# andr345/frtm-vos

Measured on AMD Instinct MI355X. Metric: segmented frames/sec/GPU (480p, ResNet101, full CG iters), higher is better.
Workload: dtype f32

## Files before the change

frtm-vos_amd/_hip.py:

```python
import ctypes
import os

import torch

_HERE = os.path.dirname(os.path.abspath(__file__))
LIB_PATH = os.path.join(_HERE, 'libfrtm_hip.so')

P, I, F, D = ctypes.c_void_p, ctypes.c_int, ctypes.c_float, ctypes.c_double


class ConvDesc(ctypes.Structure):
    _fields_ = [(k, I) for k in ('B', 'Cin', 'Hin', 'Win', 'Cout', 'ksize', 'stride', 'pad',
                                 'relu', 'out_transposed', 'splitk', 'tile', 'w_layout', 'ws_elems', 'w_pitch')]


SIGNATURES = {
    'frtm_last_error': (ctypes.c_char_p, []),
    'frtm_version': (I, []),
    'frtm_device_info': (I, [P]),
    'frtm_pixel_weights': (I, [P, I, I, I, I, F, P, P, P]),
    'frtm_normal_build': (I, [P, I, P, I, I, I, I, I, F, P, I, P, P, P, P, P]),
    'frtm_memory_next_slot': (I, [P, I, F, I, P, P, I, P]),
    'frtm_memory_insert': (I, [P, P, I, P, P]),
    'frtm_filter_scores': (I, [P, P, I, I, I, I, P, I, P]),
    'frtm_stencil': (I, [P, P, P, P, I, I, I, P, P]),
    'frtm_filter_wgrad': (I, [P, P, I, I, I, I, I, P, P]),
    'frtm_filter_wgrad_parts': (I, [I, I]),
    'frtm_filter_wgrad_parts_hw': (I, [I, I, I]),
# ... 52 lines not shown
    'frtm_backbone_set_lanes': (I, [P, I]),
    'frtm_backbone_generation': (I, [P]),
    'frtm_backbone_set_winograd': (I, [P, I]),
    'frtm_backbone_set_winograd4': (I, [P, I]),
    'frtm_backbone_set_precision': (I, [P, I]),
    'frtm_merge_masks': (I, [P, I, I, P]),
    'frtm_merge_masks_frames': (I, [P, I, I, I, P]),
    'frtm_count_above': (I, [P, I, I, F, P, P]),
    'frtm_track_merge': (I, [P, I, I, I, P, P, P, I, P, F, P]),
    'frtm_filter_scores_pitched': (I, [P, P, I, I, I, I, P, I, I, P]),
    'frtm_bilinear_resize': (I, [P, I, I, I, P, I, I, P]),
    'frtm_tse_inject': (I, [P, P, P, P, I, I, I, I, I, I, I, P, P]),
    'frtm_cab_combine': (I, [P, P, P, I, I, I, I, I, I, I, P, P]),
    'frtm_pyrup2x': (I, [P, I, I, I, P, P]),
    'frtm_plane_mean': (I, [P, I, I, P, P]),
    'frtm_conv_wgrad_ws_elems': (ctypes.c_size_t, [I, I, I, I, I, I]),
    'frtm_conv_wgrad': (I, [P, P, I, I, I, I, I, I, P, P, P, ctypes.c_size_t, P]),
    'frtm_bn_stats': (I, [P, I, I, I, F, F, I, P, P, P, P, P, P]),
    'frtm_bn_apply_relu': (I, [P, P, P, P, P, I, I, I, P, P]),
    'frtm_bn_relu_backward': (I, [P, P, P, P, P, P, I, I, I, I, P, P, P, P, P]),
    'frtm_relu_backward': (I, [P, P, ctypes.c_size_t, P, P]),
    'frtm_pyrup2x_backward': (I, [P, I, I, I, P, P, P]),
    'frtm_bilinear_backward': (I, [P, I, I, I, I, I, P, P, P]),
    'frtm_cab_backward_reduce': (I, [P, P, I, I, P, P, P]),
    'frtm_cab_gate_backward': (I, [P, P, P, P, P, P, P, P, I, I, P, P, P, P, P, P, P]),
    'frtm_cab_backward_shallow': (I, [P, P, P, I, I, P, P]),
    'frtm_add_plane': (I, [P, P, F, I, I, P]),
    'frtm_shift9': (I, [P, I, I, I, P, P]),
    'frtm_cab_gate': (I, [P, P, I, P, P, P, P, I, I, P, P]),
    'frtm_project_tail': (I, [P, I, I, I, I, P, P, I, I, P, P]),
# ... 256 lines not shown
```

frtm-vos_amd/build.py:

```python
import os
import subprocess
import sys

HERE = os.path.dirname(os.path.abspath(__file__))
CSRC = os.path.join(HERE, 'csrc')
LIB = os.path.join(HERE, 'libfrtm_hip.so')
SOURCES = ['target_model.hip', 'cg_persistent.hip', 'joint_persistent.hip', 'joint_fit.hip', 'wide_maps.hip', 'conv_igemm.hip', 'conv_gemm32.hip', 'conv_wino.hip', 'conv_wino4.hip', 'conv_bf16x3.hip', 'backbone.hip', 'image_ops.hip', 'refiner_ops.hip', 'refiner_train.hip', 'telea_host.hip', 'jf_eval.hip', 'train_step.hip', 'frame_resize.hip']
HIPCC = os.environ.get('HIPCC', '/opt/rocm/bin/hipcc')
FLAGS = ['--offload-arch=gfx950', '-O3', '-std=c++17', '-fPIC', '-Wall', '-Wno-unused-function']
if os.environ.get('FRTM_BUILD_ABLATE'):
    FLAGS.append('-DFRTM_DEBUG_ABLATE')


def _stale(target, deps):
    if not os.path.exists(target):
        return True
    t = os.path.getmtime(target)
    return any(os.path.getmtime(d) > t for d in deps)


def build(force=False, verbose=True):
    headers = [os.path.join(CSRC, 'frtm_common.h'), os.path.join(CSRC, 'conv_common.h'), os.path.join(CSRC, 'resident_grid.h'), os.path.join(os.path.dirname(HERE), 'include', 'frtm_hip.h'), __file__]
    objs = []
    for src in SOURCES:
# ... 21 lines not shown
```

frtm-vos_amd/csrc/backbone.hip:

```cpp
#include <vector>
#include <algorithm>
#include <mutex>
#include <chrono>
#include <cstdio>
#include "frtm_common.h"
#include "../../include/frtm_hip.h"

void frtm_conv_plan(int M, int Ntot, int nchunks, int vec1x1, int* tile, int* splitk);

struct ConvL {
  int Cout, Cin, ks, stride, pad;
  float* wT = nullptr; float* scale = nullptr; float* shift = nullptr; int* ktab = nullptr;
  float* wW = nullptr;
  float* wW4 = nullptr;
  float* wW6 = nullptr;
  float* wB = nullptr;
  bool loaded = false;
  int layout = 0;
  int plan_tile = 0, plan_splitk = 0;
};
struct BlockL { int conv[3]; int nconv; int ds; };

struct Lane {
  float* buf[6] = {nullptr, nullptr, nullptr, nullptr, nullptr, nullptr};
// ... 132 lines not shown
static bool bf16x3_packs(const ConvL& c) { return bf16x3_eligible(c) && c.Cin == 512 && c.Cout == 2048; }
static bool bf16x3_route(const ConvL& c, int B, int Ho, int Wo) { return bf16x3_packs(c) && (long)B * Ho * Wo >= 3240; }

static int pack_bf16x3(ConvL& c, hipStream_t st) {
  if (!c.wB) FRTM_HIP(hipMalloc((void**)&c.wB, FRTM_CONV_BF16X3_ELEMS(c.Cout, c.Cin) * sizeof(float)));
  return frtm_bf16x3_pack(c.wT, c.Cout, c.Cin, 1, (c.Cout + 31) / 32 * 32, c.wB, st);
}

static int run_conv(frtm_backbone* bb, Lane& ln, int idx, int B, int Hin, int Win, const float* in, const float* residual, int relu,
                    float* out, int* Ho, int* Wo, hipStream_t st, int pad_override = -1) {
  ConvL& c = bb->convs[idx];
  if (!c.loaded) { frtm_set_error("backbone: conv %d has no weights (call frtm_backbone_set_conv)", idx); return FRTM_ERR_STATE; }
  const int pad = pad_override >= 0 ? pad_override : c.pad;
  frtm_conv_desc d;
  d.B = B; d.Cin = c.Cin; d.Hin = Hin; d.Win = Win; d.Cout = c.Cout; d.ksize = c.ks; d.stride = c.stride; d.pad = pad;
  d.relu = relu; d.out_transposed = 0; d.splitk = 0; d.tile = 0; d.w_pitch = 0; d.w_layout = c.layout; d.ws_elems = 0;
  *Ho = (Hin + 2 * pad - c.ks) / c.stride + 1;
  *Wo = (Win + 2 * pad - c.ks) / c.stride + 1;
  {
    const size_t out_elems = (size_t)c.Cout * B * (*Ho) * (*Wo);
    const size_t w = std::min((size_t)FRTM_CONV_MAX_SPLITK * out_elems, (size_t)16 * 1024 * 1024);
    int rc = ensure(bb, &ln.ws, &ln.ws_elems, std::max(w, out_elems * 2));
    if (rc) return rc;
  }
  d.ws_elems = (int)std::min<size_t>(ln.ws_elems, 0x7fffffff);
  bb->last_launches += 1;
  bb->last_flops += 2.0 * c.Cout * (double)B * (*Ho) * (*Wo) * c.Cin * c.ks * c.ks;
  if (c.wW4 && bb->use_winograd && bb->use_winograd4) {
    int best_m = 0; long best_cost = 0, best_T = 0, best_Tp = 0;
    for (int m : {6, 4}) {
      if (m == 6 && (bb->use_winograd4 < 2 || !c.wW6)) continue;
// ... 418 lines not shown
```

frtm-vos_amd/csrc/conv_common.h:

```cpp
#pragma once
#include "frtm_common.h"

typedef float f32x4 __attribute__((ext_vector_type(4)));
typedef float f32x4u __attribute__((ext_vector_type(4), aligned(4)));

struct FastDiv { unsigned m = 1, s = 0; };
static inline FastDiv fast_div(unsigned d) {
  FastDiv f;
  unsigned s = 0;
  while ((1ull << s) < d) ++s;
  f.s = s;
  f.m = (unsigned)(((((1ull << s) - d) << 32) / d) + 1);
  return f;
}

struct ConvParams {
  const float* in; const float* wT; const int* ktab; const float* scale; const float* shift;
  const float* residual; float* out; float* ws;
  int B, Cin, Hin, Win, M, Mp, Ho, Wo, K, stride, pad;
  int Npix, Ntot, relu, out_transposed, splitk, chunks_per_split, nchunks;
  unsigned in_bytes, w_bytes;
  int w_img_stride = 0;
  int epi_pre = 1;
  FastDiv dNpix, dWo, dMt;
  FastDiv dA, dB;
  int ntiles = 0;
};

#ifdef __HIPCC__
__device__ __forceinline__ int fdiv(int n, FastDiv f) { return (int)((__umulhi((unsigned)n, f.m) + (unsigned)n) >> f.s); }
#endif
static inline void fill_divs(ConvParams& p, int bm) {
  p.dNpix = fast_div((unsigned)p.Npix);
  p.dWo = fast_div((unsigned)p.Wo);
  p.dMt = fast_div((unsigned)((p.M + bm - 1) / bm));
}

void conv_trace_reset();
void conv_trace(const char* fmt, ...) __attribute__((format(printf, 1, 2)));

constexpr int BK = 32;
// ... 41 lines not shown
```

frtm-vos_amd/csrc/conv_igemm.hip:

```cpp
#include <algorithm>
#include <atomic>
#include <cstdarg>
#include <cstdio>
#include <cstdlib>
#include "frtm_common.h"
#include "../../include/frtm_hip.h"

#include "conv_common.h"

int frtm_wino_pack(const float* w_oihw, int Cout, int Cin, float* wT, hipStream_t st);
int frtm_wino_launch(ConvParams& p, int variant, hipStream_t st);
int frtm_wino4_pack(const float* w_oihw, int Cout, int Cin, float* U, int m, hipStream_t st);
int frtm_wino4_launch(const ConvParams& p, float* ws, size_t ws_elems, int tile, int m, hipStream_t st);
int frtm_g32_launch(const ConvParams& p, int tile, hipStream_t st);
int frtm_bf16x3_pack(const float* src, int Cout, int Cin, int sm, int sk, float* out, hipStream_t st);
int frtm_bf16x3_launch(ConvParams p, hipStream_t st);

static thread_local char t_conv_trace[256];
static thread_local int t_conv_trace_len = 0;
void conv_trace_reset() { t_conv_trace_len = 0; t_conv_trace[0] = 0; }
void conv_trace(const char* fmt, ...) {
  char name[96];
  va_list ap;
  va_start(ap, fmt);
// ... 884 lines not shown
                const float* residual, float* out, float* workspace, frtm_stream_t stream) {
  conv_trace_reset();
  FRTM_CHECK_ARG(d && in && wT && out, "frtm_conv2d: null pointer");
  FRTM_CHECK_ARG(d->B > 0 && d->Cin > 0 && d->Cout > 0 && d->ksize > 0 && d->stride > 0 && d->pad >= 0, "frtm_conv2d: bad shape");
  FRTM_CHECK_ARG((scale == nullptr) == (shift == nullptr), "frtm_conv2d: scale and shift go together");
  ConvParams p;
  p.in = in; p.wT = wT; p.ktab = ktab; p.scale = scale; p.shift = shift; p.residual = residual; p.out = out; p.ws = workspace;
  p.B = d->B; p.Cin = d->Cin; p.Hin = d->Hin; p.Win = d->Win; p.M = d->Cout; p.stride = d->stride; p.pad = d->pad;
  p.Ho = (d->Hin + 2 * d->pad - d->ksize) / d->stride + 1;
  p.Wo = (d->Win + 2 * d->pad - d->ksize) / d->stride + 1;
  FRTM_CHECK_ARG(p.Ho > 0 && p.Wo > 0, "frtm_conv2d: empty output");
  p.K = d->Cin * d->ksize * d->ksize;
  p.Npix = p.Ho * p.Wo;
  p.Ntot = d->B * p.Npix;
  p.relu = d->relu; p.out_transposed = d->out_transposed;
  static const bool no_epipre = getenv("FRTM_NO_EPIPRE") != nullptr;
  p.epi_pre = no_epipre ? 0 : 1;
  p.nchunks = ceil_div(p.K, BK);
  p.Mp = (p.M + 31) / 32 * 32;
  size_t w_bytes = (size_t)p.nchunks * BK * p.Mp * 4;
  if (d->w_pitch > 0) {
    FRTM_CHECK_ARG(d->w_pitch >= p.M && d->w_pitch % 4 == 0 && ((size_t)wT) % 16 == 0,
                   "frtm_conv2d: w_pitch must be >= Cout, a multiple of 4, and wT 16-byte aligned (got %d)", d->w_pitch);
    p.Mp = d->w_pitch;
    w_bytes = (size_t)p.K * p.Mp * 4;
  }
  const size_t in_bytes = (size_t)d->B * d->Cin * d->Hin * d->Win * 4;
  FRTM_CHECK_ARG(in_bytes < 0x7fffffffull && w_bytes < 0x7fffffffull, "frtm_conv2d: tensor too large for 32-bit buffer offsets");
  p.in_bytes = (unsigned)in_bytes; p.w_bytes = (unsigned)w_bytes;
  if (d->w_layout == FRTM_WLAYOUT_WINO3X3) {
// ... 122 lines not shown
```

frtm-vos_amd/csrc/conv_wino.hip:

```cpp
#include <algorithm>
#include <cstdlib>
#include <type_traits>
#include "frtm_common.h"
#include "../../include/frtm_hip.h"
#include "conv_common.h"

#ifdef FRTM_DEBUG_TRACE
__device__ unsigned long long* g_ktw_buf = nullptr;
__device__ unsigned g_ktw_cap = 0;
__device__ unsigned g_ktw_n[288];
#define KTW_STAMP(i) do { if (threadIdx.x == 0) kt[i] = wall_clock64(); } while (0)
#else
#define KTW_STAMP(i) do { } while (0)
#endif
#if defined(FRTM_DEBUG_TRACE) && FRTM_DEBUG_TRACE >= 2
#define KTW_IN(i) do { __builtin_amdgcn_sched_barrier(0); const unsigned long long t_ = __builtin_amdgcn_s_memrealtime(); kt_in[i] += t_ - kt_last; kt_last = t_; __builtin_amdgcn_sched_barrier(0); } while (0)
#define KTW_EPI(i) do { __builtin_amdgcn_sched_barrier(0); ke[i] = __builtin_amdgcn_s_memrealtime(); __builtin_amdgcn_sched_barrier(0); } while (0)
#else
#define KTW_IN(i) do { } while (0)
#define KTW_EPI(i) do { } while (0)
#endif

constexpr int WCI = 8;
constexpr int WBM = 32;
// ... 172 lines not shown
  for (; kc + 4 <= nch; kc += 2) {
    chunk(kc, st, I0{}, I2{}); st = st == 2 ? 0 : st + 1;
    chunk(kc + 1, st, I1{}, I2{}); st = st == 2 ? 0 : st + 1;
  }
  chunk(kc, st, I0{}, I1{}); st = st == 2 ? 0 : st + 1;
  chunk(kc + 1, st, I1{}, I0{});

  constexpr int TW = BW / 2, TH = BH / 2, TILES = TW * TH;
  const int tx = tid % TW, ty = (tid / TW) % TH, cq = tid / TILES;
  const int ej = FN == 2 ? (TALL ? ty >> 2 : tx >> 2) : 0, eli = (ty & 3) * 4 + (tx & 3);
  const int mm0 = m0 + cq * CQ;
  const int xx = x0 + 2 * tx, yy0 = y0 + 2 * ty;
  const bool two = xx + 1 < p.Wo;
  const size_t img_off = (size_t)img * p.M * p.Npix;
  const unsigned out_bytes = (unsigned)p.M * (unsigned)p.Npix * 4u;
  const __amdgpu_buffer_rsrc_t rout = __builtin_amdgcn_make_buffer_rsrc((void*)(p.out + img_off), 0, (int)out_bytes, 0x00020000);
  const __amdgpu_buffer_rsrc_t rres = __builtin_amdgcn_make_buffer_rsrc(p.residual ? (void*)(p.residual + img_off) : (void*)p.out, 0,
                                                                        p.residual ? (int)out_bytes : 0, 0x00020000);
  const bool pairs = (p.Wo & 1) == 0 && (((size_t)p.out) % 8 == 0) && (!p.residual || ((size_t)p.residual) % 8 == 0);
  unsigned eo[CQ][2];
#pragma unroll
  for (int c = 0; c < CQ; ++c)
#pragma unroll
    for (int a = 0; a < 2; ++a)
      eo[c][a] = (mm0 + c < p.M && yy0 + a < p.Ho && xx < p.Wo) ? (unsigned)(((mm0 + c) * p.Npix + (yy0 + a) * p.Wo + xx) * 4) : OOB;
  f32x2 rv[CQ][2];
  __builtin_amdgcn_sched_barrier(0);
  if (pairs) {
#pragma unroll
    for (int c = 0; c < CQ; ++c)
#pragma unroll
      for (int a = 0; a < 2; ++a) rv[c][a] = __builtin_bit_cast(f32x2, __builtin_amdgcn_raw_buffer_load_b64(rres, (int)eo[c][a], 0, 0));
  } else {
#pragma unroll
// ... 100 lines not shown
  }
}

int frtm_wino_pack(const float* w_oihw, int Cout, int Cin, float* wT, hipStream_t st) {
  const size_t total = (size_t)ceil_div(Cin, WCI) * WCI * ceil_div(Cout, WBM) * WBM;
  k_pack_weights_wino<<<(int)std::min((total + 255) / 256, (size_t)2048), 256, 0, st>>>(w_oihw, Cout, Cin, wT);
  conv_trace("k_pack_weights_wino");
  FRTM_LAUNCH_CHECK();
  return FRTM_OK;
}

int frtm_wino_launch(ConvParams& p, int variant, hipStream_t st) {
  p.nchunks = ceil_div(p.Cin, WCI);
  p.w_bytes = (unsigned)((size_t)p.nchunks * ceil_div(p.M, WBM) * WFRAG * 4);
  p.splitk = 1;
  const int mt = ceil_div(p.M, WBM);
  auto padded = [&](int bh, int bw) { return (long)ceil_div(p.Ho, bh) * bh * ceil_div(p.Wo, bw) * bw; };
  if (variant == 0) {
    const long a1 = padded(8, 8), a2 = padded(8, 16), a3 = padded(16, 8);
    variant = a2 <= a3 ? 2 : 3;
    const long a = variant == 2 ? a2 : a3;
    const long blocks2 = (long)p.B * (a / 128) * mt;
    if (mt > 2 || a * 100 > a1 * 115 || blocks2 < (mt == 1 ? 512 : 1024)) variant = 1;
  }
  p.dMt = fast_div((unsigned)mt);
  { const int bh = variant == 3 ? 16 : 8, bw = variant == 2 ? 16 : 8;
    p.dA = fast_div((unsigned)(ceil_div(p.Ho, bh) * ceil_div(p.Wo, bw))); p.dB = fast_div((unsigned)ceil_div(p.Wo, bw)); }
  if (variant == 2) {
    k_conv3x3_wino<2, 0, 3><<<p.B * ceil_div(p.Ho, 8) * ceil_div(p.Wo, 16) * mt, 256, 0, st>>>(p);
    conv_trace("k_conv3x3_wino<2,0,3>");
// ... 27 lines not shown
```

frtm-vos_amd/model/seg_network.py:

```python
import torch
from torch import nn
from torch.nn import functional as F

from .. import _hip as H
from .. import ops
from ..lib.utils import conv, relu, interpolate


def _bicubic_phase(d):
    x = (d + torch.arange(-1, 3, dtype=torch.float32)).abs()
    a = -0.75
    near = (a + 2) * x ** 3 - (a + 3) * x ** 2 + 1
    far = a * x ** 3 - 5 * a * x ** 2 + 8 * a * x - 4 * a
    return torch.where(x < 1, near, torch.where(x < 2, far, torch.zeros_like(x)))


_SIDE = {}


def _shared_side_stream(dev):
    key = torch.device(dev).index
    if key not in _SIDE:
        _SIDE[key] = torch.cuda.Stream(device=dev)
    return _SIDE[key]
# ... 112 lines not shown
        self.RRB2 = nn.ModuleDict()
        for L, fc in self.ft_channels.items():
            self.TSE[L] = TSE(fc, in_channels, out_channels)
            self.RRB1[L] = RRB(out_channels, use_bn=use_bn)
            self.CAB[L] = CAB(out_channels, L == 'layer5')
            self.RRB2[L] = RRB(out_channels, use_bn=use_bn)
        self.project = _HEADS[upsampler](out_channels)
        self.use_graphs = False
        self.parallel_eager = True
        self._graphs = {}
        self._pack_key = None
        self.use_winograd = True
        self.fuse_tail = True
        self.mix_taps = True
        self.parallel_levels = True
        self._side = None
        self._pool = None
        self._uses = {}
        self.capture_after = 1

    def invalidate(self):
        self._pack_key = None
        self._graphs = {}

    def __setattr__(self, name, value):
        if isinstance(value, nn.Module) and '_pack_key' in self.__dict__:
            self.invalidate()
        super().__setattr__(name, value)

    def _apply(self, fn, *a, **k):
        self.invalidate()
# ... 79 lines not shown

    def _packed(self):
        if getattr(self, '_pack_key', None) is not None:
            return self._pack
        key = tuple((p.data_ptr(), p._version) for p in list(self.parameters()) + list(self.buffers()))
        dev = next(self.parameters()).device

        def cv(m, scale=None, shift=None, relu_=False):
            wT, ktab, lay = ops.pack_weights(m.weight.data)
            cout = m.weight.shape[0]
            if shift is None:
                shift = m.bias.data.float() if m.bias is not None else None
            if shift is not None and scale is None:
                scale = torch.ones(cout, device=dev)
            wW = ops.pack_weights(m.weight.data, wino=True)[0] if m.weight.shape[2] == 3 else None
            return dict(wT=wT, ktab=ktab, lay=lay, cout=cout, k=m.weight.shape[2], scale=None if scale is None else scale.contiguous(),
                        shift=None if shift is None else shift.contiguous(), relu=relu_, wW=wW)

        def rrb(m):
            first = m.bblock[0]
            if isinstance(m.bblock[1], nn.BatchNorm2d):
                bn = m.bblock[1]
                sc = (bn.weight / torch.sqrt(bn.running_var + bn.eps)).data.float()
                sh = (sc * (first.bias.data - bn.running_mean) + bn.bias.data).float()
            else:
                sc, sh = None, None
            return dict(c1=cv(m.conv1x1), b0=cv(first, sc, sh, True), b1=cv(m.bblock[-1], relu_=True))

        P = {}
        for L in self.ft_channels:
            t = self.TSE[L]
            w0 = t.transform[0].weight.data
# ... 10 lines not shown
        if isinstance(pj, Upsampler):
            kind = 'bicubic'
        elif isinstance(pj, BackwardCompatibleUpsampler):
            kind = 'compat'
        else:
            raise TypeError('SegNetwork: no HIP path for the head %s' % type(pj).__name__)
        P['project'] = dict(kind=kind, c1=cv(pj.conv1, relu_=True), w2=pj.conv2.weight.data.contiguous(), b2=pj.conv2.bias.data,
                            eye9=torch.eye(9, device=dev).contiguous())
        self._pack, self._pack_key = P, key
        return P

    def _conv(self, x, c, residual=None):
        if c.get('wW') is not None and self.use_winograd:
            n, _, hh, ww = x.shape
            if n * ((hh + 7) // 8) * ((ww + 7) // 8) * ((c['cout'] + 31) // 32) >= 512:
                return ops.conv2d(x, c['wW'], c['cout'], 3, 1, 1, scale=c['scale'], shift=c['shift'], residual=residual,
                                  relu=c['relu'], splitk=1, w_layout=2)
        return ops.conv2d(x, c['wT'], c['cout'], c['k'], 1, c['k'] // 2, ktab=c['ktab'], scale=c['scale'], shift=c['shift'],
                          residual=residual, relu=c['relu'], w_layout=c['lay'])

    def _rrb_hip(self, x, r):
        a = self._conv(x, r['c1'])
        return self._conv(self._conv(a, r['b0']), r['b1'], residual=a)

    @staticmethod
    def _mean(x):
        n, c, hh, ww = x.shape
        out = torch.empty(n, c, device=x.device)
        H.call('frtm_plane_mean', H.ptr(x), n * c, hh * ww, H.ptr(out))
        return out

    def _branch(self, L, p, ft, scores, deepest):
        N, _, sh, sw = scores.shape
        F_, Hh, Ww = ft.shape[0], ft.shape[-2], ft.shape[-1]
# ... 9 lines not shown
        return r, self._mean(r), pool0, (h, base, t0, t)

    def _forward_hip(self, scores, features, image_size, side_streams=None):
        P = self._packed()
        scores = scores.float().contiguous()
        n = scores.shape[0]
        frames = features[next(iter(self.ft_channels))].shape[0]
        if n % frames != 0:
            raise ValueError('scores (%d samples) must hold the same number of objects for each of the %d frames' % (n, frames))
        group = n // frames
        dev = scores.device
        levels = list(self.ft_channels)
        cur = torch.cuda.current_stream()
        keep, br = [], {}
        self._capture_events = []

        def order(waiter, waited):
            ev = torch.cuda.Event()
            ev.record(waited)
            waiter.wait_event(ev)
            self._capture_events.append(ev)
        for st in set(side_streams or []):
            order(st, cur)
        for i, L in enumerate(levels):
            ft = features[L].contiguous()
            st = side_streams[i] if (side_streams and i < len(side_streams)) else None
            if st is None:
                br[L] = self._branch(L, P[L], ft, scores, i == 0)
            else:
                with torch.cuda.stream(st):
                    br[L] = self._branch(L, P[L], ft, scores, i == 0)
        x, pool0 = None, br[levels[0]][2]
        for i, L in enumerate(levels):
            p = P[L]
            st = side_streams[i] if (side_streams and i < len(side_streams)) else None
            if st is not None:
                order(cur, st)
            r, sp, _, tmp = br[L]
            keep.append(tmp)
            Hh, Ww = r.shape[-2:]
            dp = pool0 if x is None else self._mean(x)
            gate = torch.empty(n, r.shape[1], device=dev)
            H.call('frtm_cab_gate', H.ptr(sp), H.ptr(dp), group if x is None else 0, H.ptr(p['cab_w1']), H.ptr(p['cab_b1']),
                   H.ptr(p['cab_w2']), H.ptr(p['cab_b2']), n, r.shape[1], H.ptr(gate))
            out = torch.empty_like(r)
            if x is None:
                H.call('frtm_cab_combine', H.ptr(r), H.ptr(gate), H.ptr(pool0), n, r.shape[1], 1, 1, group, Hh, Ww, H.ptr(out))
            else:
                H.call('frtm_cab_combine', H.ptr(r), H.ptr(gate), H.ptr(x), n, r.shape[1], x.shape[2], x.shape[3], 0, Hh, Ww, H.ptr(out))
            keep.append((x, gate, out, dp))
            x = self._rrb_hip(out, p['rrb2'])
        pj = P['project']
        if pj['kind'] == 'bicubic':
            return self._head_bicubic(x, pj, image_size)
        c, hh, ww = x.shape[1:]
        u1 = torch.empty(n, c, 2 * hh, 2 * ww, device=dev)
        H.call('frtm_pyrup2x', H.ptr(x), n * c, hh, ww, H.ptr(u1))
        y = self._conv(u1, pj['c1'])
        c2 = y.shape[1]
        Ho, Wo = int(image_size[-2]), int(image_size[-1])
        if self.fuse_tail and int(18 * 4.0 * hh / Ho) + 3 <= 22 and int(66 * 4.0 * ww / Wo) + 3 <= 76:
            out = torch.empty(n, 1, Ho, Wo, device=dev)
            if self.mix_taps and c2 > 9:
                ym = torch.empty(n, 9, 2 * hh, 2 * ww, device=dev)
                H.call('frtm_tap_mix', H.ptr(y), n, c2, 4 * hh * ww, H.ptr(pj['w2']), H.ptr(ym))
                H.call('frtm_project_tail', H.ptr(ym), n, 9, 2 * hh, 2 * ww, H.ptr(pj['eye9']), H.ptr(pj['b2']), Ho, Wo, H.ptr(out))
# ... 39 lines not shown
```

frtm-vos_amd/ops.py:

```python
import ctypes

import torch

from . import _hip as H

_workspaces = {}


def workspace(device, elems):
    if torch.cuda.is_current_stream_capturing():
        return torch.empty(int(elems), device=device, dtype=torch.float32)
    key = (device, H.stream())
    w = _workspaces.get(key)
    if w is None or w.numel() < elems:
        w = torch.empty(int(elems), device=device, dtype=torch.float32)
        _workspaces[key] = w
    return w


def padded_rows(K):
    return (K + 31) // 32 * 32


def padded_cols(M):
# ... 13 lines not shown
        return wT, None, 5
    layout = 4 if wino6 else 3 if wino4 else 2 if wino else (1 if (halo if halo is not None else k == 3) else 0)
    rows = 64 * padded_rows(Cin) if layout == 4 else 36 * padded_rows(Cin) if layout == 3 else max(padded_rows(Cin * k * k), (Cin + 7) // 8 * 72) if layout != 2 else (Cin + 7) // 8 * 128
    wT = torch.zeros(rows, padded_cols(Cout), device=w.device)
    ktab = torch.empty(Cin * k * k * 3, device=w.device, dtype=torch.int32) if (k > 1 and layout == 0) else None
    H.call('frtm_conv_pack_weights', H.ptr(w), Cout, Cin, k, layout, H.ptr(wT), H.ptr(ktab))
    return wT, ktab, layout


def wino4_workspace(B, Cin, Cout, Hh, Ww, device, m=4):
    tiles = (B * ((Hh + m - 1) // m) * ((Ww + m - 1) // m) + 63) // 64 * 64
    return torch.empty((m + 2) ** 2 * (Cin + Cout) * tiles, device=device)


def conv2d(x, wT, Cout, ksize=1, stride=1, pad=0, ktab=None, scale=None, shift=None, residual=None, relu=False,
           out=None, out_transposed=False, splitk=0, tile=0, shape=None, w_pitch=0, w_layout=0, ws=None):
    B, Cin, Hin, Win = shape if shape is not None else x.shape
    Ho = (Hin + 2 * pad - ksize) // stride + 1
    Wo = (Win + 2 * pad - ksize) // stride + 1
    if out is None:
        out = torch.empty((B, Ho * Wo, Cout) if out_transposed else (B, Cout, Ho, Wo), device=x.device, dtype=torch.float32)
    out_elems = Cout * B * Ho * Wo
    if ws is None and splitk != 1:
        ws = workspace(x.device, min(32 * out_elems, max(2 * out_elems, 1 << 24)))
    d = H.ConvDesc(B, Cin, Hin, Win, Cout, ksize, stride, pad, int(relu), int(out_transposed), int(splitk), int(tile), int(w_layout),
                   0 if ws is None else min(ws.numel(), 0x7fffffff), int(w_pitch))
    H.call('frtm_conv2d', ctypes.byref(d), H.ptr(x), H.ptr(wT), H.ptr(ktab), H.ptr(scale), H.ptr(shift),
           H.ptr(residual), H.ptr(out), H.ptr(ws))
    return out


def filter_scores(X, f, out=None, accumulate=False, n=None, interleave=None):
    N = X.shape[0] if n is None else n
    C, h, w = X.shape[1:]
    if interleave is not None:
        batch, k, groups = interleave
        assert batch.is_contiguous() and batch.shape[0] == N * groups and tuple(batch.shape[-2:]) == (h, w)
        H.call('frtm_filter_scores_pitched', H.ptr(X), H.ptr(f), N, C, h, w, batch.data_ptr() + 4 * k * h * w, groups * h * w, int(accumulate))
        return batch
    if out is None:
        out = torch.empty(N, 1, h, w, device=X.device)
    H.call('frtm_filter_scores', H.ptr(X), H.ptr(f), N, C, h, w, H.ptr(out), int(accumulate))
    return out

# ... 236 lines not shown
```

include/frtm_hip.h:

```cpp
#ifndef FRTM_HIP_H
#define FRTM_HIP_H

#ifdef __cplusplus
extern "C" {
#endif

typedef void* frtm_stream_t;
typedef struct frtm_backbone frtm_backbone_t;

const char* frtm_last_error(void);
int frtm_version(void);
int frtm_device_info(int* out4_host);


#define FRTM_PX_PARTS 32
int frtm_pixel_weights(const void* y, int y_is_u8, int n, int H, int W, float tf,
                       float* out, float* scratch, frtm_stream_t stream);

int frtm_normal_build(const void* labels, int labels_is_u8, const float* pw, int n, int H, int W, int h, int w,
                      float tf, const int* slot_dev, int slot_host, float* Bmem, float* cmem,
                      float* scratch, const int* px_count_dev, frtm_stream_t stream);

int frtm_memory_update_window(float* sw, int cap, float lr, int num_samp_is_zero, int* state, const int* counts, int count_stride,
                              int min_count, int W, int* slots, const float* features, float* samples, int len, const float* labels,
// ... 77 lines not shown
int frtm_joint_run_persistent(const float* X, const float* Z, const float* Bm, const float* cm, const float* sw, int N, int Cin, int c, int h, int w,
                              const float* w1T, float* w1, float* w2, float* vec, float* state, float* scratch, unsigned* bar, unsigned* hbar,
                              int iters, int has_p, int apply_dff, int fletcher_reeves, int standard_alpha, float dff, float lam1, float lam2,
                              float invM1, float invM2, float step, unsigned* stats, int debug_abort, frtm_stream_t stream);
int frtm_vec_axpy(float* y, float a, const float* x, int n, frtm_stream_t stream);
int frtm_transpose2d(const float* in, int rows, int cols, float* out, frtm_stream_t stream);

typedef struct {
  int B, Cin, Hin, Win, Cout, ksize, stride, pad;
  int relu, out_transposed;
  int splitk;
  int tile;
  int w_layout;
  int ws_elems;
  int w_pitch;
} frtm_conv_desc;
#define FRTM_CONV_MAX_SPLITK 32
#define FRTM_WLAYOUT_GEMM 0
#define FRTM_WLAYOUT_HALO3X3 1
#define FRTM_WLAYOUT_WINO3X3 2
#define FRTM_CONV_WINO_ELEMS(Cout, Cin) ((((Cin) + 7) / 8 * 128) * (((Cout) + 31) / 32 * 32))
#define FRTM_WLAYOUT_WINO4 3
#define FRTM_CONV_WINO4_ELEMS(Cout, Cin) (36 * (((Cin) + 31) / 32 * 32) * (((Cout) + 31) / 32 * 32))
#define FRTM_CONV_WINO4_TILES(B, H, W) ((((B) * (((H) + 3) / 4) * (((W) + 3) / 4)) + 63) / 64 * 64)
#define FRTM_CONV_WINO4_WS_ELEMS(B, Cin, Cout, H, W) ((size_t)36 * ((Cin) + (Cout)) * FRTM_CONV_WINO4_TILES(B, H, W))
#define FRTM_WLAYOUT_WINO6 4
#define FRTM_CONV_WINO6_ELEMS(Cout, Cin) (64 * (((Cin) + 31) / 32 * 32) * (((Cout) + 31) / 32 * 32))
#define FRTM_CONV_WINO6_TILES(B, H, W) ((((B) * (((H) + 5) / 6) * (((W) + 5) / 6)) + 63) / 64 * 64)
#define FRTM_CONV_WINO6_WS_ELEMS(B, Cin, Cout, H, W) ((size_t)64 * ((Cin) + (Cout)) * FRTM_CONV_WINO6_TILES(B, H, W))
#define FRTM_WLAYOUT_BF16X3 5
// ... 58 lines not shown

int frtm_bilinear_resize(const float* in, int planes, int h, int w, float* out, int H, int W, frtm_stream_t stream);
int frtm_tse_inject(const float* base, const float* bias, const float* ws, const float* scores, int n, int group, int C,
                    int h, int w, int H, int W, float* out, frtm_stream_t stream);
int frtm_cab_combine(const float* shallow, const float* gate, const float* deeper, int n, int C, int hd, int wd, int deeper_group,
                     int H, int W, float* out, frtm_stream_t stream);
int frtm_cab_gate(const float* sp, const float* dp, int dp_group, const float* W1, const float* b1, const float* W2, const float* b2,
                  int n, int oc, float* gate, frtm_stream_t stream);
int frtm_pyrup2x(const float* in, int planes, int h, int w, float* out, frtm_stream_t stream);
int frtm_project_tail(const float* y, int n, int C, int h, int w, const float* w3x3, const float* bias, int Ho, int Wo, float* out,
                      frtm_stream_t stream);
int frtm_tap_mix(const float* y, int n, int C, int hw, const float* w3x3, float* out, frtm_stream_t stream);
int frtm_bicubic_resize(const float* in, int planes, int h, int w, float* out, int H, int W, frtm_stream_t stream);
int frtm_project_tail_bicubic(const float* y, int n, int C, int h, int w, const float* w3x3, const float* bias, int Ho, int Wo, float* out,
                              frtm_stream_t stream);
int frtm_plane_mean(const float* in, int planes, int HW, float* out, frtm_stream_t stream);

size_t frtm_conv_wgrad_ws_elems(int B, int Cout, int Cin, int k, int H, int W);
int frtm_conv_wgrad(const float* dy, const float* x, int B, int Cout, int Cin, int k, int H, int W, float* dw, float* dbias, float* ws,
                    size_t ws_elems, frtm_stream_t stream);
int frtm_bn_stats(const float* x, int N, int C, int HW, float eps, float factor, int train, float* rmean, float* rvar, float* mean,
                  float* invstd, double* part, frtm_stream_t stream);
int frtm_bn_apply_relu(const float* x, const float* mean, const float* invstd, const float* gamma, const float* beta, int N, int C, int HW,
                       float* out, frtm_stream_t stream);
int frtm_bn_relu_backward(const float* dy, const float* out, const float* x, const float* mean, const float* invstd, const float* gamma,
                          int N, int C, int HW, int train, float* dx, float* dgamma, float* dbeta, double* part, frtm_stream_t stream);
int frtm_relu_backward(const float* dy, const float* y, size_t n, float* dx, frtm_stream_t stream);
int frtm_pyrup2x_backward(const float* dout, int planes, int h, int w, float* din, float* tmp, frtm_stream_t stream);
int frtm_bilinear_backward(const float* dout, int planes, int h, int w, int H, int W, float* din, float* tmp, frtm_stream_t stream);
int frtm_cab_backward_reduce(const float* dout, const float* shallow, int planes, int HW, float* a, float* b, frtm_stream_t stream);
// ... 61 lines not shown
```

Before: 662.4.

## Split odd output channel of Winograd 3x3 convs into a dedicated plane kernel

For 3x3 Winograd convs whose Cout is one more than a multiple of 32 (e.g. 33), the main Winograd GEMM now computes only Cout-1 channels and writes them with a strided per-image output. A new single-plane Winograd F(2x2,3x3) kernel, which shares horizontal neighbours across lanes with DPP, computes the leftover channel, so the GEMM no longer pads a whole 32-wide M tile for one channel. The segmentation decoder is also reordered so refinement tails for earlier levels run on side streams before the join. This adds an out_img_stride field to the conv descriptor ABI, an extra launch per split conv, and more cross-stream event ordering.

```diff
diff --git a/frtm-vos_amd/_hip.py b/frtm-vos_amd/_hip.py
--- a/frtm-vos_amd/_hip.py
+++ b/frtm-vos_amd/_hip.py
@@ -12,6 +12,13 @@
 class ConvDesc(ctypes.Structure):
     _fields_ = [(k, I) for k in ('B', 'Cin', 'Hin', 'Win', 'Cout', 'ksize', 'stride', 'pad',
                                  'relu', 'out_transposed', 'splitk', 'tile', 'w_layout', 'ws_elems', 'w_pitch')]
+
+    def __new__(cls, *a, **k):
+        return super().__new__(ConvDescStrided if cls is ConvDesc else cls, *a, **k)
+
+
+class ConvDescStrided(ConvDesc):
+    _fields_ = [('out_img_stride', I)]
 
 
 SIGNATURES = {
@@ -94,6 +101,7 @@
     'frtm_cab_combine': (I, [P, P, P, I, I, I, I, I, I, I, P, P]),
     'frtm_pyrup2x': (I, [P, I, I, I, P, P]),
     'frtm_plane_mean': (I, [P, I, I, P, P]),
+    'frtm_conv3x3_plane': (I, [P, I, I, I, I, P, P, P, I, P, ctypes.c_size_t, P]),
     'frtm_conv_wgrad_ws_elems': (ctypes.c_size_t, [I, I, I, I, I, I]),
     'frtm_conv_wgrad': (I, [P, P, I, I, I, I, I, I, P, P, P, ctypes.c_size_t, P]),
     'frtm_bn_stats': (I, [P, I, I, I, F, F, I, P, P, P, P, P, P]),
diff --git a/frtm-vos_amd/build.py b/frtm-vos_amd/build.py
--- a/frtm-vos_amd/build.py
+++ b/frtm-vos_amd/build.py
@@ -5,7 +5,7 @@
 HERE = os.path.dirname(os.path.abspath(__file__))
 CSRC = os.path.join(HERE, 'csrc')
 LIB = os.path.join(HERE, 'libfrtm_hip.so')
-SOURCES = ['target_model.hip', 'cg_persistent.hip', 'joint_persistent.hip', 'joint_fit.hip', 'wide_maps.hip', 'conv_igemm.hip', 'conv_gemm32.hip', 'conv_wino.hip', 'conv_wino4.hip', 'conv_bf16x3.hip', 'backbone.hip', 'image_ops.hip', 'refiner_ops.hip', 'refiner_train.hip', 'telea_host.hip', 'jf_eval.hip', 'train_step.hip', 'frame_resize.hip']
+SOURCES = ['target_model.hip', 'cg_persistent.hip', 'joint_persistent.hip', 'joint_fit.hip', 'wide_maps.hip', 'conv_igemm.hip', 'conv_gemm32.hip', 'conv_wino.hip', 'conv_wino4.hip', 'conv_bf16x3.hip', 'conv_plane.hip', 'backbone.hip', 'image_ops.hip', 'refiner_ops.hip', 'refiner_train.hip', 'telea_host.hip', 'jf_eval.hip', 'train_step.hip', 'frame_resize.hip']
 HIPCC = os.environ.get('HIPCC', '/opt/rocm/bin/hipcc')
 FLAGS = ['--offload-arch=gfx950', '-O3', '-std=c++17', '-fPIC', '-Wall', '-Wno-unused-function']
 if os.environ.get('FRTM_BUILD_ABLATE'):
diff --git a/frtm-vos_amd/csrc/backbone.hip b/frtm-vos_amd/csrc/backbone.hip
--- a/frtm-vos_amd/csrc/backbone.hip
+++ b/frtm-vos_amd/csrc/backbone.hip
@@ -170,7 +170,7 @@
   const int pad = pad_override >= 0 ? pad_override : c.pad;
   frtm_conv_desc d;
   d.B = B; d.Cin = c.Cin; d.Hin = Hin; d.Win = Win; d.Cout = c.Cout; d.ksize = c.ks; d.stride = c.stride; d.pad = pad;
-  d.relu = relu; d.out_transposed = 0; d.splitk = 0; d.tile = 0; d.w_pitch = 0; d.w_layout = c.layout; d.ws_elems = 0;
+  d.relu = relu; d.out_transposed = 0; d.splitk = 0; d.tile = 0; d.w_pitch = 0; d.w_layout = c.layout; d.ws_elems = 0; d.out_img_stride = 0;
   *Ho = (Hin + 2 * pad - c.ks) / c.stride + 1;
   *Wo = (Win + 2 * pad - c.ks) / c.stride + 1;
   {
diff --git a/frtm-vos_amd/csrc/conv_common.h b/frtm-vos_amd/csrc/conv_common.h
--- a/frtm-vos_amd/csrc/conv_common.h
+++ b/frtm-vos_amd/csrc/conv_common.h
@@ -25,6 +25,7 @@
   FastDiv dNpix, dWo, dMt;
   FastDiv dA, dB;
   int ntiles = 0;
+  int out_img_stride = 0;
 };
 
 #ifdef __HIPCC__
diff --git a/frtm-vos_amd/csrc/conv_igemm.hip b/frtm-vos_amd/csrc/conv_igemm.hip
--- a/frtm-vos_amd/csrc/conv_igemm.hip
+++ b/frtm-vos_amd/csrc/conv_igemm.hip
@@ -922,6 +922,14 @@
   p.Npix = p.Ho * p.Wo;
   p.Ntot = d->B * p.Npix;
   p.relu = d->relu; p.out_transposed = d->out_transposed;
+  if (d->out_img_stride != 0) {
+    FRTM_CHECK_ARG(d->w_layout == FRTM_WLAYOUT_WINO3X3 && !d->out_transposed && d->splitk <= 1,
+                   "frtm_conv2d: out_img_stride needs the Winograd F(2x2,3x3) layout (no GEMM, halo, three-launch Winograd, G32, bf16x3, split-K or transposed launch)");
+    FRTM_CHECK_ARG(!residual, "frtm_conv2d: out_img_stride does not go with a residual (the residual is read densely)");
+    FRTM_CHECK_ARG(d->out_img_stride >= d->Cout * p.Npix && (size_t)d->Cout * p.Npix < 0x20000000ull,
+                   "frtm_conv2d: out_img_stride (%d floats) is smaller than one image's output (%d x %d)", d->out_img_stride, d->Cout, p.Npix);
+    p.out_img_stride = d->out_img_stride;
+  }
   static const bool no_epipre = getenv("FRTM_NO_EPIPRE") != nullptr;
   p.epi_pre = no_epipre ? 0 : 1;
   p.nchunks = ceil_div(p.K, BK);
diff --git a/frtm-vos_amd/csrc/conv_plane.hip b/frtm-vos_amd/csrc/conv_plane.hip
--- /dev/null
+++ b/frtm-vos_amd/csrc/conv_plane.hip
@@ -0,0 +1,140 @@
+#include "frtm_common.h"
+#include "../../include/frtm_hip.h"
+#include "conv_common.h"
+
+typedef float f32x2p __attribute__((ext_vector_type(2)));
+
+__device__ __forceinline__ float lane_below(float v) {
+  return __builtin_bit_cast(float, __builtin_amdgcn_update_dpp(0, __builtin_bit_cast(int, v), 0x138, 0xf, 0xf, false));
+}
+__device__ __forceinline__ float lane_above(float v) {
+  return __builtin_bit_cast(float, __builtin_amdgcn_update_dpp(0, __builtin_bit_cast(int, v), 0x130, 0xf, 0xf, false));
+}
+
+template <int VEC>
+__global__ __launch_bounds__(256) void k_conv3x3_plane(const float* __restrict__ in, const float* __restrict__ U, const float* __restrict__ scale,
+                                                        const float* __restrict__ shift, int relu, int Cin, int H, int W, int TW, int THW, int total,
+                                                        unsigned in_bytes, float* __restrict__ out, size_t out_img_stride) {
+  const int lane = threadIdx.x & 63, wave = blockIdx.x * 4 + (threadIdx.x >> 6);
+  if (wave * 62 >= total) return;
+  const int q = wave * 62 + lane - 1;
+  const bool inside = q >= 0 && q < total;
+  const int HW = H * W;
+  const int n = inside ? q / THW : 0, rem = q - n * THW, ty = inside ? rem / TW : 0, tx = rem - ty * TW, y0 = 2 * ty, x0 = 2 * tx;
+  const __amdgpu_buffer_rsrc_t rin = __builtin_amdgcn_make_buffer_rsrc((void*)in, 0, (int)in_bytes, 0x00020000);
+  unsigned off[4], off1[4];
+  const bool has1 = x0 + 1 < W;
+#pragma unroll
+  for (int r = 0; r < 4; ++r) {
+    const int yy = y0 + r - 1;
+    const bool ok = inside && (unsigned)yy < (unsigned)H;
+    off[r] = ok ? ((unsigned)n * (unsigned)Cin * (unsigned)HW + (unsigned)(yy * W + x0)) * 4u : OOB;
+    off1[r] = (ok && has1) ? off[r] + 4u : OOB;
+  }
+  const bool lz = x0 == 0, rz = x0 + 2 >= W;
+  float acc[4][4];
+#pragma unroll
+  for (int r = 0; r < 4; ++r)
+#pragma unroll
+    for (int c = 0; c < 4; ++c) acc[r][c] = 0.f;
+  auto channel = [&](int ci, const float* c1, const float* c2) {
+    float u[4][4];
+    {
+      float d[4][4];
+#pragma unroll
+      for (int r = 0; r < 4; ++r) {
+        const float a = lane_below(c2[r]), b = lane_above(c1[r]);
+        d[r][0] = lz ? 0.f : a; d[r][1] = c1[r]; d[r][2] = c2[r]; d[r][3] = rz ? 0.f : b;
+      }
+#pragma unroll
+      for (int c = 0; c < 4; ++c) {
+        u[0][c] = d[0][c] - d[2][c];
+        u[1][c] = d[1][c] + d[2][c];
+        u[2][c] = d[2][c] - d[1][c];
+        u[3][c] = d[1][c] - d[3][c];
+      }
+    }
+    const float* Uc = U + ci * 16;
+#pragma unroll
+    for (int r = 0; r < 4; ++r) {
+      const float v0 = u[r][0] - u[r][2], v1 = u[r][1] + u[r][2], v2 = u[r][2] - u[r][1], v3 = u[r][1] - u[r][3];
+      acc[r][0] = __builtin_fmaf(Uc[r * 4 + 0], v0, acc[r][0]);
+      acc[r][1] = __builtin_fmaf(Uc[r * 4 + 1], v1, acc[r][1]);
+      acc[r][2] = __builtin_fmaf(Uc[r * 4 + 2], v2, acc[r][2]);
+      acc[r][3] = __builtin_fmaf(Uc[r * 4 + 3], v3, acc[r][3]);
+    }
+  };
+  constexpr int CU = 4;
+  int ci = 0;
+  for (; ci + CU <= Cin; ci += CU) {
+    float c1[CU][4], c2[CU][4];
+#pragma unroll
+    for (int k = 0; k < CU; ++k)
+#pragma unroll
+      for (int r = 0; r < 4; ++r) {
+        const unsigned cstep = (unsigned)(ci + k) * (unsigned)HW * 4u;
+        if constexpr (VEC == 2) {
+          const f32x2p v = __builtin_bit_cast(f32x2p, __builtin_amdgcn_raw_buffer_load_b64(rin, (int)off[r], (int)cstep, 0));
+          c1[k][r] = v.x; c2[k][r] = v.y;
+        } else {
+          c1[k][r] = buf_ld1s(rin, off[r], cstep); c2[k][r] = buf_ld1s(rin, off1[r], cstep);
+        }
+      }
+#pragma unroll
+    for (int k = 0; k < CU; ++k) channel(ci + k, c1[k], c2[k]);
+  }
+  for (; ci < Cin; ++ci) {
+    float c1[4], c2[4];
+    const unsigned cstep = (unsigned)ci * (unsigned)HW * 4u;
+#pragma unroll
+    for (int r = 0; r < 4; ++r) {
+      if constexpr (VEC == 2) {
+        const f32x2p v = __builtin_bit_cast(f32x2p, __builtin_amdgcn_raw_buffer_load_b64(rin, (int)off[r], (int)cstep, 0));
+        c1[r] = v.x; c2[r] = v.y;
+      } else {
+        c1[r] = buf_ld1s(rin, off[r], cstep); c2[r] = buf_ld1s(rin, off1[r], cstep);
+      }
+    }
+    channel(ci, c1, c2);
+  }
+  if (!inside || lane == 0 || lane == 63) return;
+  float P[4][2];
+#pragma unroll
+  for (int r = 0; r < 4; ++r) {
+    P[r][0] = acc[r][0] + acc[r][1] + acc[r][2];
+    P[r][1] = acc[r][1] - acc[r][2] - acc[r][3];
+  }
+  const float sc = scale ? scale[0] : 1.f, sh = shift ? shift[0] : 0.f;
+  float* o = out + (size_t)n * out_img_stride + (size_t)y0 * W + x0;
+#pragma unroll
+  for (int a = 0; a < 2; ++a)
+#pragma unroll
+    for (int b = 0; b < 2; ++b) {
+      float v = a == 0 ? P[0][b] + P[1][b] + P[2][b] : P[1][b] - P[2][b] - P[3][b];
+      v = __builtin_fmaf(v, sc, sh);
+      if (relu) v = fmaxf(v, 0.f);
+      if (y0 + a < H && x0 + b < W) o[(size_t)a * W + b] = v;
+    }
+}
+
+extern "C" {
+
+int frtm_conv3x3_plane(const float* in, int n, int Cin, int H, int W, const float* U, const float* scale, const float* shift, int relu,
+                       float* out, size_t out_img_stride, frtm_stream_t stream) {
+  conv_trace_reset();
+  FRTM_CHECK_ARG(in && U && out && n > 0 && Cin > 0 && H > 0 && W > 0, "frtm_conv3x3_plane: bad argument");
+  FRTM_CHECK_ARG((size_t)n * Cin * H * W * 4 < 0x7fffffffull, "frtm_conv3x3_plane: input too large for 32-bit buffer offsets");
+  FRTM_CHECK_ARG(out_img_stride >= (size_t)H * W, "frtm_conv3x3_plane: out_img_stride is smaller than one plane");
+  const int TW = ceil_div(W, 2), THW = ceil_div(H, 2) * TW, total = n * THW;
+  const unsigned in_bytes = (unsigned)((size_t)n * Cin * H * W * 4);
+  const dim3 g(ceil_div(ceil_div(total, 62), 4));
+  hipStream_t st = (hipStream_t)stream;
+  const bool vec = (W % 2 == 0) && ((size_t)in % 8 == 0);
+  if (vec) k_conv3x3_plane<2><<<g, 256, 0, st>>>(in, U, scale, shift, relu, Cin, H, W, TW, THW, total, in_bytes, out, out_img_stride);
+  else k_conv3x3_plane<1><<<g, 256, 0, st>>>(in, U, scale, shift, relu, Cin, H, W, TW, THW, total, in_bytes, out, out_img_stride);
+  conv_trace("k_conv3x3_plane<%d>", vec ? 2 : 1);
+  FRTM_LAUNCH_CHECK();
+  return FRTM_OK;
+}
+
+}
diff --git a/frtm-vos_amd/csrc/conv_wino.hip b/frtm-vos_amd/csrc/conv_wino.hip
--- a/frtm-vos_amd/csrc/conv_wino.hip
+++ b/frtm-vos_amd/csrc/conv_wino.hip
@@ -210,10 +210,10 @@
   const bool two = xx + 1 < p.Wo;
   const size_t img_off = (size_t)img * p.M * p.Npix;
   const unsigned out_bytes = (unsigned)p.M * (unsigned)p.Npix * 4u;
-  const __amdgpu_buffer_rsrc_t rout = __builtin_amdgcn_make_buffer_rsrc((void*)(p.out + img_off), 0, (int)out_bytes, 0x00020000);
+  const __amdgpu_buffer_rsrc_t rout = __builtin_amdgcn_make_buffer_rsrc((void*)(p.out + (size_t)img * p.out_img_stride), 0, (int)out_bytes, 0x00020000);
   const __amdgpu_buffer_rsrc_t rres = __builtin_amdgcn_make_buffer_rsrc(p.residual ? (void*)(p.residual + img_off) : (void*)p.out, 0,
                                                                         p.residual ? (int)out_bytes : 0, 0x00020000);
-  const bool pairs = (p.Wo & 1) == 0 && (((size_t)p.out) % 8 == 0) && (!p.residual || ((size_t)p.residual) % 8 == 0);
+  const bool pairs = (p.Wo & 1) == 0 && (p.out_img_stride & 1) == 0 && (((size_t)p.out) % 8 == 0) && (!p.residual || ((size_t)p.residual) % 8 == 0);
   unsigned eo[CQ][2];
 #pragma unroll
   for (int c = 0; c < CQ; ++c)
@@ -344,6 +344,7 @@
   p.nchunks = ceil_div(p.Cin, WCI);
   p.w_bytes = (unsigned)((size_t)p.nchunks * ceil_div(p.M, WBM) * WFRAG * 4);
   p.splitk = 1;
+  if (p.out_img_stride == 0) p.out_img_stride = p.M * p.Npix;
   const int mt = ceil_div(p.M, WBM);
   auto padded = [&](int bh, int bw) { return (long)ceil_div(p.Ho, bh) * bh * ceil_div(p.Wo, bw) * bw; };
   if (variant == 0) {
diff --git a/frtm-vos_amd/model/seg_network.py b/frtm-vos_amd/model/seg_network.py
--- a/frtm-vos_amd/model/seg_network.py
+++ b/frtm-vos_amd/model/seg_network.py
@@ -150,7 +150,12 @@
         self.fuse_tail = True
         self.mix_taps = True
         self.parallel_levels = True
+        self.split_odd_channel = True
+        self.split_min_pixels = 60000
+        self.plane_on_side = False
+        self.side_tails = True
         self._side = None
+        self._capture_events = []
         self._pool = None
         self._uses = {}
         self.capture_after = 1
@@ -260,8 +265,14 @@
             if shift is not None and scale is None:
                 scale = torch.ones(cout, device=dev)
             wW = ops.pack_weights(m.weight.data, wino=True)[0] if m.weight.shape[2] == 3 else None
-            return dict(wT=wT, ktab=ktab, lay=lay, cout=cout, k=m.weight.shape[2], scale=None if scale is None else scale.contiguous(),
-                        shift=None if shift is None else shift.contiguous(), relu=relu_, wW=wW)
+            d = dict(wT=wT, ktab=ktab, lay=lay, cout=cout, k=m.weight.shape[2], scale=None if scale is None else scale.contiguous(),
+                     shift=None if shift is None else shift.contiguous(), relu=relu_, wW=wW)
+            if wW is not None and cout > 32 and cout % 32 == 1:
+                w = m.weight.data.float()
+                d['split'] = dict(wW=ops.pack_weights(w[:cout - 1], wino=True)[0], w=ops.plane_weights(w[cout - 1]),
+                                  scale=None if scale is None else scale[:cout - 1].contiguous(), shift=None if shift is None else shift[:cout - 1].contiguous(),
+                                  scale1=None if scale is None else scale[cout - 1:].contiguous(), shift1=None if shift is None else shift[cout - 1:].contiguous())
+            return d
 
         def rrb(m):
             first = m.bblock[0]
@@ -302,10 +313,38 @@
         if c.get('wW') is not None and self.use_winograd:
             n, _, hh, ww = x.shape
             if n * ((hh + 7) // 8) * ((ww + 7) // 8) * ((c['cout'] + 31) // 32) >= 512:
+                sp = c.get('split')
+                if sp is not None and self.split_odd_channel and residual is None and n * hh * ww >= self.split_min_pixels:
+                    return self._conv_split(x, c, sp)
                 return ops.conv2d(x, c['wW'], c['cout'], 3, 1, 1, scale=c['scale'], shift=c['shift'], residual=residual,
                                   relu=c['relu'], splitk=1, w_layout=2)
         return ops.conv2d(x, c['wT'], c['cout'], c['k'], 1, c['k'] // 2, ktab=c['ktab'], scale=c['scale'], shift=c['shift'],
                           residual=residual, relu=c['relu'], w_layout=c['lay'])
+
+    def _conv_split(self, x, c, sp):
+        n, _, hh, ww = x.shape
+        cout = c['cout']
+        out = torch.empty(n, cout, hh, ww, device=x.device)
+        stride = cout * hh * ww
+        cur = torch.cuda.current_stream()
+        side = self._side[0] if (self.plane_on_side and self._side and not torch.cuda.is_current_stream_capturing()) else None
+        if side is not None and side != cur:
+            self._order(side, cur)
+            with torch.cuda.stream(side):
+                ops.conv3x3_plane(x, sp['w'], out[0, cout - 1], stride, scale=sp['scale1'], shift=sp['shift1'], relu=c['relu'])
+        ops.conv2d(x, sp['wW'], cout - 1, 3, 1, 1, scale=sp['scale'], shift=sp['shift'], relu=c['relu'], splitk=1, w_layout=2,
+                   out=out, out_img_stride=stride)
+        if side is not None and side != cur:
+            self._order(cur, side)
+        else:
+            ops.conv3x3_plane(x, sp['w'], out[0, cout - 1], stride, scale=sp['scale1'], shift=sp['shift1'], relu=c['relu'])
+        return out
+
+    def _order(self, waiter, waited):
+        ev = torch.cuda.Event()
+        ev.record(waited)
+        waiter.wait_event(ev)
+        self._capture_events.append(ev)
 
     def _rrb_hip(self, x, r):
         a = self._conv(x, r['c1'])
@@ -345,28 +384,16 @@
         cur = torch.cuda.current_stream()
         keep, br = [], {}
         self._capture_events = []
-
-        def order(waiter, waited):
-            ev = torch.cuda.Event()
-            ev.record(waited)
-            waiter.wait_event(ev)
-            self._capture_events.append(ev)
+        order = self._order
         for st in set(side_streams or []):
             order(st, cur)
-        for i, L in enumerate(levels):
-            ft = features[L].contiguous()
-            st = side_streams[i] if (side_streams and i < len(side_streams)) else None
-            if st is None:
-                br[L] = self._branch(L, P[L], ft, scores, i == 0)
-            else:
-                with torch.cuda.stream(st):
-                    br[L] = self._branch(L, P[L], ft, scores, i == 0)
-        x, pool0 = None, br[levels[0]][2]
-        for i, L in enumerate(levels):
-            p = P[L]
-            st = side_streams[i] if (side_streams and i < len(side_streams)) else None
-            if st is not None:
-                order(cur, st)
+        pool0 = None
+        state = dict(x=None, on=cur)
+
+        def tail(L, on):
+            p, x = P[L], state['x']
+            if x is not None and state['on'] != on:
+                order(on, state['on'])
             r, sp, _, tmp = br[L]
             keep.append(tmp)
             Hh, Ww = r.shape[-2:]
@@ -380,7 +407,39 @@
             else:
                 H.call('frtm_cab_combine', H.ptr(r), H.ptr(gate), H.ptr(x), n, r.shape[1], x.shape[2], x.shape[3], 0, Hh, Ww, H.ptr(out))
             keep.append((x, gate, out, dp))
-            x = self._rrb_hip(out, p['rrb2'])
+            state['x'], state['on'] = self._rrb_hip(out, p['rrb2']), on
+
+        early = bool(side_streams) and self.side_tails
+        pending = []
+        for i, L in enumerate(levels):
+            ft = features[L].contiguous()
+            st = side_streams[i] if (side_streams and i < len(side_streams)) else None
+            if st is None:
+                br[L] = self._branch(L, P[L], ft, scores, i == 0)
+            else:
+                with torch.cuda.stream(st):
+                    br[L] = self._branch(L, P[L], ft, scores, i == 0)
+                    if i == 0:
+                        pool0 = br[L][2]
+                    if early and i < len(levels) - 1 and not pending:
+                        tail(L, st)
+                        continue
+            if i == 0:
+                pool0 = br[L][2]
+            pending.append((L, st))
+        joined = set()
+        if early:
+            for st in side_streams:
+                if st is not None and st not in joined:
+                    order(cur, st)
+                    joined.add(st)
+            if state['on'] in joined:
+                state['on'] = cur
+        for L, st in pending:
+            if st is not None and st not in joined:
+                order(cur, st)
+            tail(L, cur)
+        x = state['x']
         pj = P['project']
         if pj['kind'] == 'bicubic':
             return self._head_bicubic(x, pj, image_size)
diff --git a/frtm-vos_amd/ops.py b/frtm-vos_amd/ops.py
--- a/frtm-vos_amd/ops.py
+++ b/frtm-vos_amd/ops.py
@@ -51,7 +51,7 @@
 
 
 def conv2d(x, wT, Cout, ksize=1, stride=1, pad=0, ktab=None, scale=None, shift=None, residual=None, relu=False,
-           out=None, out_transposed=False, splitk=0, tile=0, shape=None, w_pitch=0, w_layout=0, ws=None):
+           out=None, out_transposed=False, splitk=0, tile=0, shape=None, w_pitch=0, w_layout=0, ws=None, out_img_stride=0):
     B, Cin, Hin, Win = shape if shape is not None else x.shape
     Ho = (Hin + 2 * pad - ksize) // stride + 1
     Wo = (Win + 2 * pad - ksize) // stride + 1
@@ -62,9 +62,25 @@
         ws = workspace(x.device, min(32 * out_elems, max(2 * out_elems, 1 << 24)))
     d = H.ConvDesc(B, Cin, Hin, Win, Cout, ksize, stride, pad, int(relu), int(out_transposed), int(splitk), int(tile), int(w_layout),
                    0 if ws is None else min(ws.numel(), 0x7fffffff), int(w_pitch))
+    d.out_img_stride = int(out_img_stride)
     H.call('frtm_conv2d', ctypes.byref(d), H.ptr(x), H.ptr(wT), H.ptr(ktab), H.ptr(scale), H.ptr(shift),
            H.ptr(residual), H.ptr(out), H.ptr(ws))
     return out
+
+
+def plane_weights(w_row):
+    Cin = w_row.shape[0]
+    wT = pack_weights(w_row.reshape(1, Cin, 3, 3), wino=True)[0]
+    nch = (Cin + 7) // 8
+    img = wT.flatten()[:nch * 4096].view(nch, 16, 4, 16, 2, 2)[:, :, :, 0, :, 0]
+    return img.permute(0, 3, 2, 1).reshape(nch * 8, 16)[:Cin].contiguous()
+
+
+def conv3x3_plane(x, U, out_plane, out_img_stride, scale=None, shift=None, relu=False):
+    N, Cin, Hh, Ww = x.shape
+    assert U.is_contiguous() and tuple(U.shape) == (Cin, 16)
+    H.call('frtm_conv3x3_plane', H.ptr(x), N, Cin, Hh, Ww, H.ptr(U), H.ptr(scale), H.ptr(shift), int(relu), out_plane.data_ptr(), int(out_img_stride))
+    return out_plane
 
 
 def filter_scores(X, f, out=None, accumulate=False, n=None, interleave=None):
diff --git a/include/frtm_hip.h b/include/frtm_hip.h
--- a/include/frtm_hip.h
+++ b/include/frtm_hip.h
@@ -115,6 +115,7 @@
   int w_layout;
   int ws_elems;
   int w_pitch;
+  int out_img_stride;
 } frtm_conv_desc;
 #define FRTM_CONV_MAX_SPLITK 32
 #define FRTM_WLAYOUT_GEMM 0
@@ -203,6 +204,8 @@
 int frtm_bicubic_resize(const float* in, int planes, int h, int w, float* out, int H, int W, frtm_stream_t stream);
 int frtm_project_tail_bicubic(const float* y, int n, int C, int h, int w, const float* w3x3, const float* bias, int Ho, int Wo, float* out,
                               frtm_stream_t stream);
+int frtm_conv3x3_plane(const float* in, int n, int Cin, int H, int W, const float* U, const float* scale, const float* shift, int relu,
+                       float* out, size_t out_img_stride, frtm_stream_t stream);
 int frtm_plane_mean(const float* in, int planes, int HW, float* out, frtm_stream_t stream);
 
 size_t frtm_conv_wgrad_ws_elems(int B, int Cout, int Cin, int k, int H, int W);
```

Result: no change. 668.5, median of 6 (+0.9%).
